# tky823/audio_source_separation

Measured on AMD Instinct MI355X. Metric: ILRMA iterations/sec (4ch, F=1025, T=4096), higher is better.
Workload: dtype f64; 1 GPU; gauss_ilrma_ip update_once, M=4 F=1025 T=4096 K=4, normalize=power, loss off; utterances_per_gpu=1, power_statistic=covariance, parallelism=utterance-sharded x1, no data-path collective

## Files before the change

audio_source_separation_amd/_lib.py:

```python
import ctypes
import os

import torch

_HERE = os.path.dirname(os.path.abspath(__file__))
LIB_PATH = os.environ.get("ASSX_LIB_PATH") or os.path.join(_HERE, "csrc", "libassx.so")

F32, F64 = 0, 1
W_NONE, W_NT, W_NFT = 0, 1, 2
IVA_LAPLACE, IVA_GAUSS = 0, 1
NMF_EUC, NMF_KL, NMF_IS_MM, NMF_IS_ME = 0, 1, 2, 3
NMF_T, NMF_CAUCHY_NAIVE, NMF_CAUCHY_MM, NMF_CAUCHY_ME, NMF_CAUCHY_MM_FAST = 4, 5, 6, 7, 8
STATUS_SINGULAR, STATUS_COND_REJECT = 1, 2
SPATIAL_IP, SPATIAL_ISS, SPATIAL_IP2 = 0, 1, 2

_vp = ctypes.c_void_p
_i = ctypes.c_int
_d = ctypes.c_double
_sz = ctypes.c_size_t
_ll = ctypes.c_longlong

SIGNATURES = {
    "assx_ctx_create": (_i, [_i, ctypes.POINTER(_vp)]),
    "assx_ctx_destroy": (_i, [_vp]),
    "assx_last_error": (ctypes.c_char_p, [_vp]),
    "assx_version": (ctypes.c_char_p, []),
    "assx_workspace_bytes": (_sz, [_i, _i, _i, _i, _i, _i]),
    "assx_launch_order": (_i, [_i, _i, _i, _i, _vp, _i]),
    "assx_nmf_partition_query": (_i, [_i, _i, _i, _i, _i, _i, _i, _vp]),
    "assx_demix": (_i, [_vp, _vp, _vp, _vp, _vp, _i, _i, _i, _i, _i, _vp]),
    "assx_cov_accumulate": (_i, [_vp, _vp, _vp, _i, _d, _vp, _vp, _i, _i, _i, _i, _i, _i, _vp]),
    "assx_ip_update": (_i, [_vp, _vp, _vp, _d, _vp, _i, _i, _i, _i, _vp]),
    "assx_ilrma_source_update": (_i, [_vp, _vp, _vp, _vp, _vp, _d, _d, ctypes.c_uint, _vp, _vp, _i, _i, _i, _i, _i, _i, _vp]),
    "assx_ilrma_expand_partitioned": (_i, [_vp, _vp, _vp, _vp, _vp, _vp, _i, _i, _i, _i, _i, _i, _vp]),
    "assx_ilrma_source_update_partitioned": (_i, [_vp, _vp, _vp, _vp, _vp, _vp, _vp, _vp, _d, _vp, _i, _i, _i, _i, _i, _i, _vp]),
    "assx_ilrma_normalize_power_bins_partitioned": (_i, [_vp, _vp, _vp, _vp, _vp, _d, _vp, _i, _i, _i, _i, _i, _vp]),
    "assx_ilrma_spatial_update": (_i, [_vp, _i, _i, _i, _vp, _vp, _vp, _vp, _d, _d, _d, _vp, _vp, _vp, _vp, _vp, _i, _i, _i, _i, _i, _i, _vp]),
    "assx_ip2_update": (_i, [_vp, _vp, _vp, _d, _vp, _i, _i, _i, _i, _i, _i, _vp]),
    "assx_iss_update": (_i, [_vp, _vp, _vp, _i, _i, _i, _i, _i, _vp]),
    "assx_ilrma_cov_partials": (_i, [_vp, _vp, _vp, _vp, _d, _d, _vp, _i, _i, _i, _i, _i, _i, _vp]),
    "assx_demix_power": (_i, [_vp, _vp, _vp, _vp, _vp, _i, _i, _i, _i, _i, _vp]),
    "assx_power_from_cov": (_i, [_vp, _vp, _vp, _vp, _vp, _i, _i, _i, _i, _vp]),
    "assx_ilrma_normalize_power": (_i, [_vp, _vp, _vp, _vp, _d, _d, _i, _i, _i, _i, _i, _vp]),
    "assx_ilrma_normalize_power_bins": (_i, [_vp, _vp, _vp, _vp, _d, _d, _i, _i, _i, _i, _i, _vp]),
    "assx_ilrma_normalize_pb": (_i, [_vp, _vp, _vp, _vp, _d, _i, _i, _i, _i, _i, _vp]),
    "assx_ilrma_loss": (_i, [_vp, _vp, _vp, _vp, _vp, _d, _d, _vp, _vp, _i, _i, _i, _i, _i, _i, _vp]),
    "assx_tilrma_source_update": (_i, [_vp, _vp, _vp, _vp, _vp, _d, _d, _vp, _i, _i, _i, _i, _i, _i, _vp]),
    "assx_tilrma_spatial_update": (_i, [_vp, _vp, _vp, _vp, _vp, _d, _d, _vp, _vp, _vp, _vp, _vp, _i, _i, _i, _i, _i, _i, _vp]),
    "assx_tilrma_loss": (_i, [_vp, _vp, _vp, _vp, _vp, _d, _d, _vp, _vp, _i, _i, _i, _i, _i, _i, _vp]),
    "assx_auxiva_weights": (_i, [_vp, _vp, _vp, _i, _d, _vp, _vp, _vp, _i, _i, _i, _i, _i, _vp]),
    "assx_auxiva_spatial_update": (_i, [_vp, _i, _i, _i, _vp, _vp, _vp, _d, _d, _vp, _vp, _vp, _i, _i, _i, _i, _i, _vp]),
    "assx_idlma_space_update": (_i, [_vp, _vp, _vp, _vp, _d, _d, _d, _vp, _vp, _vp, _i, _i, _i, _i, _i, _vp]),
    "assx_fastmnmf_update_diagonalizer": (_i, [_vp, _vp, _vp, _vp, _vp, _d, _d, _vp, _vp, _vp, _i, _i, _i, _i, _i, _i, _vp]),
    "assx_fastmnmf_workspace_bytes": (_sz, [_i, _i, _i, _i, _i, _i, _i]),
    "assx_fastmnmf_project": (_i, [_vp, _vp, _vp, _vp, _vp, _vp, _d, _vp, _vp, _i, _i, _i, _i, _i, _i, _i, _vp]),
    "assx_fastmnmf_update_nmf": (_i, [_vp, _vp, _vp, _vp, _d, _vp, _i, _i, _i, _i, _i, _i, _i, _vp]),
    "assx_fastmnmf_update_scm": (_i, [_vp, _vp, _vp, _vp, _d, _vp, _i, _i, _i, _i, _i, _i, _i, _vp]),
    "assx_fastmnmf_update_diagonalizer_model": (_i, [_vp, _vp, _vp, _vp, _vp, _vp, _d, _d, _vp, _vp, _i, _i, _i, _i, _i, _i,
                                                     _i, _vp]),
    "assx_fastmnmf_normalize_power": (_i, [_vp, _vp, _vp, _vp, _vp, _d, _i, _i, _i, _i, _i, _i, _i, _vp]),
    "assx_fastmnmf_separate": (_i, [_vp, _vp, _vp, _vp, _vp, _vp, _i, _d, _vp, _vp, _i, _i, _i, _i, _i, _i, _i, _vp]),
# ... 76 lines not shown
```

audio_source_separation_amd/csrc/assx_bss.hip:

```cpp
#include "assx_common.hpp"
#include "assx_small_linalg.hpp"
#include "assx_stream.hpp"
#include "assx_group_linalg.hpp"
#include "assx_partition.hpp"
#include "assx_cov_wide.hpp"
#include "assx_cov_mfma.hpp"
#include "assx_nmf_internal.hpp"
#include "assx_widem.hpp"

using namespace assx;

namespace {

constexpr int REDUCE_THREADS = 256;

template <typename R, int M>
__device__ __forceinline__ void load_filter(const Cx<R>* __restrict__ W, size_t bf, Cx<R> (&w)[M][M]) {
  const Cx<R>* p = W + bf * (M * M);
#pragma unroll
  for (int n = 0; n < M; ++n)
#pragma unroll
    for (int m = 0; m < M; ++m) w[n][m] = p[n * M + m];
}

// ... 837 lines not shown
#endif
    }
  } else if (dtype == ASSX_F32) {
#if !defined(ASSX_DEV_ONLY_M4_F64)
    switch (M) {
#if !defined(ASSX_DEV_ONLY_M4_F32)
      case 2: return fn(float(), IntC<2>());
      case 3: return fn(float(), IntC<3>());
#endif
      case 4: return fn(float(), IntC<4>());
    }
#endif
  } else {
    return fail(ctx, ASSX_E_ARG, "dtype must be ASSX_F32 or ASSX_F64, got %d", dtype);
  }
  return fail(ctx, ASSX_E_UNSUPPORTED,
              "this entry point supports 2 <= M <= 4 channels, got M=%d (5 <= M <= 32 runs on the wide-channel path of the "
              "model entry points; more than 32 channels are not supported)", M);
}

#define CHECK_COMMON(ctx, B, M, F, T)                                                        \
  ASSX_REQUIRE_CTX(ctx);                              \
  ASSX_REQUIRE(ctx, (B) >= 1 && (M) >= 1 && (F) >= 1 && (T) >= 1, ASSX_E_ARG,                 \
               "invalid sizes B=%d M=%d F=%d T=%d", (B), (M), (F), (T));                       \
  ASSX_REQUIRE(ctx, (long long)(M) * (F) * (T) < (1LL << 28) && (long long)(B) * (F) * (((T) + 31) / 32 + 1) < (1LL << 31), \
               ASSX_E_UNSUPPORTED,                                                                                       \
               "utterance too large: buffer offsets are 32-bit, one utterance must stay below 4 GiB in complex128 "     \
               "(M*F*T < 2^28) and B*F*T/32 below 2^31")

inline unsigned blocks_for(size_t n, int bs) { return (unsigned)((n + bs - 1) / bs); }

inline unsigned set_launch_order(FlatPart& fp, int B, int rev) {
  static const int on = lab_int("ASSX_UTT_ORDER", 1);
  if (!on || B < 2) {
    fp.Gp = 0;
    fp.rev = 0;
    return (unsigned)fp.G;
  }
  fp.Gp = (fp.Gu + N_XCD - 1) / N_XCD * N_XCD;
  fp.rev = rev ? 1 : 0;
  return (unsigned)B * (unsigned)fp.Gp;
}
inline unsigned stream_grid(assx_ctx* ctx, FlatPart& fp, int B) {
  return set_launch_order(fp, B, B >= 2 ? (int)(ctx->stream_pass++ & 1u) : 0);
}

template <typename R, int M>
int run_cov_partial(assx_ctx* ctx, int wk, const void* X, const void* r, const void* Tb, const void* V, int K,
                    double domain, double eps, void* ws, int B, int F, int T, hipStream_t st, FlatPart* fp_out) {
  CovArgs<R> a;
  a.d = Dims{B, F, T, K};
  a.fp = flat_cov(B, F, T, wk == WK_NONE ? 1 : cov_lane_split<R, M>());
  a.eps = (R)eps;
  a.p2d = make_pow(2.0 / domain);
  *fp_out = a.fp;
  dim3 grid(stream_grid(ctx, a.fp, B));
  const bool d2 = a.p2d.mode == POW_ID;
#define COV_LAUNCH(WKV, K4V, D2V, LSV, DXV, DWV, MW) \
  hipLaunchKernelGGL((cov_stream_kernel<R, M, WKV, K4V, D2V, LSV, DXV, DWV, MW>), grid, dim3(64), 0, st, \
                     (const Cx<R>*)X, (const R*)r, (const R*)Tb, (const R*)V, (R*)ws, a)
  constexpr int LSX = cov_lane_split<R, M>();
  switch (wk) {
    case WK_NONE: COV_LAUNCH(WK_NONE, true, true, 1, 4, 1, 1); break;
    case WK_NT: COV_LAUNCH(WK_NT, true, true, LSX, 3, 1, 2); break;
    case WK_NFT: COV_LAUNCH(WK_NFT, true, true, LSX, 3, 1, 2); break;
    default:
      if (K <= KU) {
        constexpr size_t vlds = (size_t)VDMA_SLOTS * VTileDma<R, M * KU>::TILE_BYTES;
#if ASSX_LAB
        static const int vdma = lab_int("ASSX_COV_VDMA", 1);
        if (!vdma) {
          if (d2) COV_LAUNCH(WK_TV, true, true, LSX, (sizeof(R) == 8 ? 2 : 4), 1, 2);
          else COV_LAUNCH(WK_TV, true, false, LSX, 2, 1, 1);
        } else
#endif
        if (d2)
          hipLaunchKernelGGL((cov_stream_kernel<R, M, WK_TV, true, true, 1, 2, 1, 2, true>), grid, dim3(64), vlds, st,
                             (const Cx<R>*)X, (const R*)r, (const R*)Tb, (const R*)V, (R*)ws, a);
        else
          hipLaunchKernelGGL((cov_stream_kernel<R, M, WK_TV, true, false, 1, 2, 1, 1, true>), grid, dim3(64), vlds, st,
                             (const Cx<R>*)X, (const R*)r, (const R*)Tb, (const R*)V, (R*)ws, a);
      }
      else if (d2) COV_LAUNCH(WK_TV, false, true, LSX, 4, 1, 1);
      else COV_LAUNCH(WK_TV, false, false, LSX, 2, 1, 1);
  }
#undef COV_LAUNCH
  ASSX_LAUNCH_CHECK(ctx, "cov_stream_kernel");
  return 0;
}

template <typename R, int M>
int run_cov(assx_ctx* ctx, int wk, const void* X, const void* r, const void* Tb, const void* V, int K, double domain,
            double eps, void* U, void* ws, int B, int F, int T, hipStream_t st) {
  FlatPart fp;
  int rc = run_cov_partial<R, M>(ctx, wk, X, r, Tb, V, K, domain, eps, ws, B, F, T, st, &fp);
  if (rc) return rc;
  const int N = (wk == WK_NONE) ? 1 : M;
  const size_t total = (size_t)B * N * F * M * M;
  hipLaunchKernelGGL((cov_stream_finalize_kernel<R, M>), dim3(blocks_for(total, 256)), dim3(256), 0, st, (const R*)ws,
                     (Cx<R>*)U, B, N, F, fp, (R)(1.0 / (double)T));
  ASSX_LAUNCH_CHECK(ctx, "cov_stream_finalize_kernel");
  return 0;
}

template <typename R, int M>
int run_ip(assx_ctx* ctx, const void* U, const void* part, FlatPart fp, int T, void* W, const void* C, double* pw,
           double thr, int32_t* status, int B, int F, hipStream_t st, double den_floor = 0.0, int wb = 1) {
  constexpr int GPW = WAVE / next_pow2_c(M * M);
#if ASSX_LAB
  const int par = lab_int("ASSX_IP_PAR", 0);
  if (par) {
    const dim3 gp(blocks_for((size_t)B * F, GPW / M)), bp(64);
    if (part)
      hipLaunchKernelGGL((ip_par_kernel<R, M, true>), gp, bp, 0, st, (const Cx<R>*)nullptr, (const R*)part, fp,
// ... 29 lines not shown
                       (double)T, (Cx<R>*)W, (const Cx<R>*)C, pw, B, F);
  ASSX_LAUNCH_CHECK(ctx, "iss_group_kernel");
  return 0;
}

template <typename R, int M>
int run_ip2(assx_ctx* ctx, const void* U, const void* part, FlatPart fp, int T, void* W, const void* C, double* pw,
            double thr, int32_t* status, int B, int F, int pm, int pn, hipStream_t st) {
  constexpr int GPW = WAVE / next_pow2_c(M * M);
  const dim3 grid(blocks_for((size_t)B * F, GPW)), block(64);
  if (part)
    hipLaunchKernelGGL((ip2_group_kernel<R, M, true>), grid, block, 0, st, (const Cx<R>*)nullptr, (const R*)part, fp,
                       1.0 / (double)T, (Cx<R>*)W, (const Cx<R>*)C, pw, thr, status, B, F, pm, pn);
  else
    hipLaunchKernelGGL((ip2_group_kernel<R, M, false>), grid, block, 0, st, (const Cx<R>*)U, (const R*)nullptr, fp, 1.0,
                       (Cx<R>*)W, (const Cx<R>*)C, pw, thr, status, B, F, pm, pn);
  ASSX_LAUNCH_CHECK(ctx, "ip2_group_kernel");
  return 0;
}

template <typename R, int MM>
int run_basis_partial(assx_ctx* ctx, const void* X, const void* W, const void* Tb, const void* V, double domain,
                      double eps, void* ws, int B, int F, int T, int K, hipStream_t st, FlatPart* fp_out,
                      double nu = -1.0 ,
                      double* lpart = nullptr , int lstride = 0) {
  NmfArgs<R> a;
  a.nu = (R)nu;
  a.d = Dims{B, F, T, K};
  a.eps = (R)eps;
  a.p1 = make_pow((domain + 2.0) / domain);
  a.fp = flat_basis(B, F, T);
  *fp_out = a.fp;
  const bool d2 = a.p1.mode == POW_SQUARE, k4 = K <= KU;
  const dim3 gb(stream_grid(ctx, a.fp, B)), bb(64);
#define BASIS_LAUNCH(K4V, D2V, DXV, DWV, MW) \
  hipLaunchKernelGGL((basis_stream_kernel<R, MM, K4V, D2V, DXV, DWV, MW>), gb, bb, 0, st, (const Cx<R>*)X, \
                     (const Cx<R>*)W, (const R*)Tb, (const R*)V, (R*)ws, a)
  constexpr size_t vlds = (size_t)VDMA_SLOTS * VTileDma<R, MM * KU>::TILE_BYTES;
#define BASIS_VD(D2V, MW, TDV) \
  hipLaunchKernelGGL((basis_stream_vd_kernel<R, MM, D2V, 2, MW, TDV>), gb, bb, vlds, st, (const Cx<R>*)X, \
                     (const Cx<R>*)W, (const R*)Tb, (const R*)V, (R*)ws, a, (double*)nullptr, 0)
#if ASSX_LAB
  static const int vdma = lab_int("ASSX_BASIS_VDMA", 1);
  if (k4 && !vdma) {
    if (nu >= 0.0) hipLaunchKernelGGL((basis_stream_kernel<R, MM, true, true, 3, 1, 1, true>), gb, bb, 0, st, (const Cx<R>*)X,
                                      (const Cx<R>*)W, (const R*)Tb, (const R*)V, (R*)ws, a);
    else if (d2) BASIS_LAUNCH(true, true, 3, 1, 2);
    else BASIS_LAUNCH(true, false, 2, 1, 1);
  } else
#endif
  if (nu >= 0.0) {
    if (k4) BASIS_VD(true, 2, true);
    else hipLaunchKernelGGL((basis_stream_kernel<R, MM, false, true, 3, 1, 1, true>), gb, bb, 0, st, (const Cx<R>*)X,
                            (const Cx<R>*)W, (const R*)Tb, (const R*)V, (R*)ws, a);
  } else if (k4) {
    if (d2 && lpart)
      hipLaunchKernelGGL((basis_stream_vd_kernel<R, MM, true, 2, 2, false, true>), gb, bb, vlds, st, (const Cx<R>*)X,
                         (const Cx<R>*)W, (const R*)Tb, (const R*)V, (R*)ws, a, lpart, lstride);
    else if (d2) BASIS_VD(true, 2, false);
    else BASIS_VD(false, 1, false);
  } else if (d2) BASIS_LAUNCH(false, true, 3, 1, 1);
  else BASIS_LAUNCH(false, false, 2, 1, 1);
#undef BASIS_VD
#undef BASIS_LAUNCH
  ASSX_LAUNCH_CHECK(ctx, "basis_stream_kernel");
  return 0;
}

template <typename R, int MM>
int run_act_partial(assx_ctx* ctx, const void* X, const void* W, const void* Tb, const void* V, double domain,
                    double eps, void* ws, int B, int F, int T, int K, hipStream_t st, FlatPart* fp_out,
                    double nu = -1.0) {
  NmfArgs<R> a;
  a.nu = (R)nu;
  a.d = Dims{B, F, T, K};
  a.eps = (R)eps;
  a.p1 = make_pow((domain + 2.0) / domain);
  a.fp = flat_act(B, F, T);
  *fp_out = a.fp;
  const bool d2 = a.p1.mode == POW_SQUARE, k4 = K <= KU;
  const dim3 ga(stream_grid(ctx, a.fp, B)), ba(64 * ACT_NH);
#define ACT_LAUNCH(K4V, D2V, DXV, MW) \
  hipLaunchKernelGGL((act_stream_kernel<R, MM, K4V, D2V, DXV, MW>), ga, ba, 0, st, (const Cx<R>*)X, (const Cx<R>*)W, \
                     (const R*)Tb, (const R*)V, (R*)ws, a)
#define ACT_VD(D2V, DXV, MW, TDV) \
  hipLaunchKernelGGL((act_stream_vd_kernel<R, MM, D2V, DXV, MW, TDV>), ga, ba, 0, st, (const Cx<R>*)X, (const Cx<R>*)W, \
                     (const R*)Tb, (const R*)V, (R*)ws, a)
#if ASSX_LAB
  static const int vdma = lab_int("ASSX_ACT_VDMA", 1);
  if (k4 && !vdma) {
    if (nu >= 0.0) hipLaunchKernelGGL((act_stream_kernel<R, MM, true, true, 3, 1, true>), ga, ba, 0, st, (const Cx<R>*)X,
                                      (const Cx<R>*)W, (const R*)Tb, (const R*)V, (R*)ws, a);
    else if (d2) ACT_LAUNCH(true, true, (sizeof(R) == 8 ? 3 : 4), 2);
    else ACT_LAUNCH(true, false, 2, 1);
  } else
#endif
// ... 92 lines not shown
      *fp_out = fw;
      return 0;
    }
    hipLaunchKernelGGL((cov_wide_finalize_kernel<R, MM>), dim3(blocks_for((size_t)B * MM * F * MM * MM, 256)), dim3(256),
                       0, st, (const R*)ws, (Cx<R>*)U_dense, B, F, fw, (R)(1.0 / (double)T));
    ASSX_LAUNCH_CHECK(ctx, "cov_wide_finalize_kernel");
    *fp_out = fw;
    *dense = true;
    return 0;
  }
  R* rv = (R*)((char*)ws + L.map);
  const dim3 grid(blocks_for(T, 256), blocks_for(F, WIDE_FB), B * MM);
  if (p2d.mode == POW_ID)
    hipLaunchKernelGGL((source_variance_map_kernel<R, true>), grid, dim3(256), 0, st, (const R*)Tb, (const R*)V, rv, F, T,
                       K, p2d);
  else
    hipLaunchKernelGGL((source_variance_map_kernel<R, false>), grid, dim3(256), 0, st, (const R*)Tb, (const R*)V, rv, F,
                       T, K, p2d);
  ASSX_LAUNCH_CHECK(ctx, "source_variance_map_kernel");
  return run_cov_partial<R, MM>(ctx, WK_NFT, X, rv, nullptr, nullptr, 1, 2.0, eps, ws, B, F, T, st, fp_out);
}

}

extern "C" {

int assx_launch_order(int B, int F, int T, int reverse, int* ranges, int capacity) {
  if (B < 1 || F < 1 || T < 1) return ASSX_E_ARG;
  FlatPart fp = flat_cov(B, F, T, 1);
  const int grid = (int)set_launch_order(fp, B, reverse);
  if (ranges) {
    if (capacity < grid) return ASSX_E_ARG;
    for (int bid = 0; bid < grid; ++bid) ranges[bid] = workgroup_range(bid, grid, fp);
  }
  return grid;
}

size_t assx_workspace_bytes(int B, int M, int F, int T, int K, int dtype) {
  if (B < 1 || M < 1 || F < 1 || T < 1) return 0;
  if (widem::handles(M)) return widem::workspace_bytes(B, M, F, T, K, dtype);
  return ws_layout(B, M, F, T, K, dtype).total;
}

int assx_demix(assx_ctx* ctx, const void* X, const void* W, const void* scale, void* Y, int B, int M, int F, int T,
               int dtype, void* stream) {
  CHECK_COMMON(ctx, B, M, F, T);
  ASSX_REQUIRE(ctx, X && W && Y, ASSX_E_NULL, "assx_demix: NULL array");
  if (widem::handles(M)) return widem::demix(ctx, X, W, scale, Y, B, M, F, T, dtype, (hipStream_t)stream);
  hipStream_t st = (hipStream_t)stream;
  return dispatch_rm(ctx, dtype, M, [&](auto rt, auto mt) -> int {
    using R = decltype(rt);
    constexpr int MM = decltype(mt)::value;
    dim3 grid(blocks_for(T, 256), F, B);
    hipLaunchKernelGGL((demix_kernel<R, MM>), grid, dim3(256), 0, st, (const Cx<R>*)X, (const Cx<R>*)W,
                       (const Cx<R>*)scale, (Cx<R>*)Y, Dims{B, F, T, 0});
    ASSX_LAUNCH_CHECK(ctx, "demix_kernel");
    return 0;
  });
}

int assx_ilrma_power_map(assx_ctx* ctx, const void* X, const void* W, void* P, int B, int M, int F, int T, int dtype,
                         void* stream) {
  CHECK_COMMON(ctx, B, M, F, T);
  ASSX_REQUIRE(ctx, X && W && P, ASSX_E_NULL, "assx_ilrma_power_map: NULL array");
  hipStream_t st = (hipStream_t)stream;
  if (widem::handles(M)) return widem::power_map(ctx, X, W, P, B, M, F, T, dtype, st);
// ... 877 lines not shown
```

audio_source_separation_amd/csrc/assx_stream.hpp:

```cpp
#pragma once
#include <cstdlib>
#include "assx_common.hpp"

namespace assx {

enum { WK_NONE = 0, WK_NT = 1, WK_NFT = 2, WK_TV = 3 };

constexpr int KU = 4;

struct Dims {
  int B, F, T, K;
};

struct FlatPart {
  long long NB;
  int len;
  int L;
  int G;
  int S;
  int Gu;
  int Ju;
  int P;
  int Gp;
  int rev;
};

inline FlatPart make_flat(int B, long long NB, int len, long long G_target) {
  FlatPart p;
  p.Gp = 0;
  p.rev = 0;
  p.NB = NB;
  p.len = len;
  p.Ju = (int)(NB / len);
  p.P = 0;
  long long G = G_target < NB ? G_target : NB;
  if (G < 1) G = 1;
  const long long parts = G / p.Ju;
  static const bool align = lab_int("ASSX_ALIGN", 1) != 0;
  if (align && parts >= 1 && parts <= len && p.Ju * parts * 100 >= G * 97) {
    p.L = (int)((len + parts - 1) / parts);
    p.P = (len + p.L - 1) / p.L;
    p.Gu = p.Ju * p.P;
    p.G = B * p.Gu;
    p.S = 1;
    return p;
  }
  p.L = (int)((NB + G - 1) / G);
  p.Gu = (int)((NB + p.L - 1) / p.L);
  p.G = B * p.Gu;
  p.S = (p.L + len - 2) / len + 1;
  return p;
}

__host__ __device__ __forceinline__ bool flat_local(const FlatPart& fp, unsigned gl, unsigned& lo, unsigned& n) {
  const unsigned L = (unsigned)fp.L;
  if (fp.P > 0) {
    const unsigned grp = gl / (unsigned)fp.P, part = gl - grp * (unsigned)fp.P, len = (unsigned)fp.len;
    const unsigned off = part * L;
    if (off >= len) return false;
    lo = grp * len + off;
    n = off + L < len ? L : len - off;
    return true;
  }
// ... 28 lines not shown
    g_hi = g_lo + (fp.len + fp.L - 1) / fp.L - 1;
    return;
  }
  const unsigned lo = jl * (unsigned)fp.len;
  g_lo = b * fp.Gu + (int)(lo / (unsigned)fp.L);
  g_hi = b * fp.Gu + (int)((lo + (unsigned)fp.len - 1u) / (unsigned)fp.L);
}
__host__ __device__ __forceinline__ int flat_slot(const FlatPart& fp, long long j, int g) {
  if (fp.P > 0) return 0;
  const int b = g / fp.Gu, gl = g - b * fp.Gu;
  return (int)(j - (long long)b * fp.Ju) - (int)(((unsigned)gl * (unsigned)fp.L) / (unsigned)fp.len);
}

struct Cursor {
  int b, f, tb;
};
__device__ __forceinline__ void advance(Cursor& c, int TBk, int F) {
  if (++c.tb == TBk) {
    c.tb = 0;
    if (++c.f == F) {
      c.f = 0;
      ++c.b;
    }
  }
}

constexpr int N_XCD = 8;
__host__ __device__ __forceinline__ int xcd_local_range(int bid, int G) {
  const int x = bid % N_XCD, j = bid / N_XCD;
  const int q = G / N_XCD, r = G % N_XCD;
  return x * q + (x < r ? x : r) + j;
}

__host__ __device__ __forceinline__ int workgroup_range(int bid, int grid, const FlatPart& fp) {
  if (fp.Gp == 0) return xcd_local_range(bid, grid);
  const int Gp = fp.Gp, B = grid / Gp;
  int b = bid / Gp;
  const int r = bid - b * Gp;
  const int x = r % N_XCD, j = r / N_XCD;
  const int q = fp.Gu / N_XCD, rem = fp.Gu % N_XCD;
  const int cnt = q + (x < rem ? 1 : 0);
  if (j >= cnt) return -1;
  const int first = x * q + (x < rem ? x : rem);
  if (fp.rev) {
    b = B - 1 - b;
    return b * fp.Gu + first + (cnt - 1 - j);
  }
  return b * fp.Gu + first + j;
}


template <typename R, int NROW>
struct VTileDma {
  static constexpr int LPR = WAVE * (int)sizeof(R) / 16;
  static constexpr int RPI = WAVE / LPR;
  static constexpr int NI = NROW / RPI;
  static constexpr int ROW_BYTES = WAVE * (int)sizeof(R);
  static constexpr int TILE_BYTES = NROW * ROW_BYTES;
  static constexpr int NP = NROW / 2;
  static_assert(NROW % RPI == 0 && NROW % 2 == 0 && (NP == 4 || NP == 6 || NP == 8), "tile geometry");
  unsigned vro[NI];

  __device__ __forceinline__ void init(int lane, int K, unsigned t_row) {
    const int grp = lane / LPR, piece = lane % LPR;
#pragma unroll
    for (int j = 0; j < NI; ++j) {
      const int rho = j * RPI + grp;
      const int n = rho / KU, kk = rho % KU;
      vro[j] = (unsigned)(n * K + (kk < K ? kk : K - 1)) * t_row + (unsigned)piece * 16u;
    }
  }
  __device__ __forceinline__ void issue(BufRsrc rv, unsigned char* slot, unsigned soff) const {
#if defined(__HIP_DEVICE_COMPILE__)
#pragma unroll
    for (int j = 0; j < NI; ++j)
      __builtin_amdgcn_raw_ptr_buffer_load_lds(rv, (__attribute__((address_space(3))) void*)(slot + j * RPI * ROW_BYTES),
                                               16, (int)vro[j], (int)soff, 0, 0);
#endif
  }
};

// ... 58 lines not shown
      "ds_read2st64_b32 %0, %4 offset0:0 offset1:1\n\tds_read2st64_b32 %1, %4 offset0:2 offset1:3\n\t"
      "ds_read2st64_b32 %2, %4 offset0:4 offset1:5\n\tds_read2st64_b32 %3, %4 offset0:6 offset1:7\n\t"
      "s_waitcnt lgkmcnt(0)"
      : "=&v"(o[0]), "=&v"(o[1]), "=&v"(o[2]), "=&v"(o[3])
      : "v"(addr)
      : "memory");
}

constexpr int VDMA_SLOTS = 2;

template <int M>
__host__ __device__ constexpr int herm_pair_base(int m, int l) {
  return M + 2 * (m * M - m * (m + 1) / 2 + (l - m - 1));
}

template <typename R>
struct CovArgs {
  Dims d;
  FlatPart fp;
  R eps;
  PowSpec p2d;
};

#ifndef STREAM_TRACE
#define STREAM_TRACE 0
#endif
#if STREAM_TRACE && !defined(ASSX_PROBE_BUILD)
#error "STREAM_TRACE adds a debug entry point and stamps: build it with -DASSX_PROBE_BUILD into a probe library, never into libassx.so"
#endif
#if STREAM_TRACE
__device__ unsigned long long g_stream_trace[8 * 4096];
#endif

template <typename R, int M, int WK, bool K4, bool D2, int LS, int DXT, int DWT, int MINW = 1, bool VDMA = false>
__global__ void __launch_bounds__(64, MINW)
    cov_stream_kernel(const Cx<R>* __restrict__ X, const R* __restrict__ rw ,
                      const R* __restrict__ Tb , const R* __restrict__ V ,
                      R* __restrict__ part, CovArgs<R> a) {
  constexpr int N = (WK == WK_NONE) ? 1 : M;
  static_assert(N % LS == 0 && DXT % DWT == 0, "lane split / ring depths");
  constexpr int FB = WAVE / LS;
  constexpr int SPL = N / LS;
  constexpr int HM = M * M;
  constexpr int NACC = SPL * HM;
  constexpr int NV = next_pow2_c(NACC);
  static_assert(NV <= FB, "accumulators per lane must not exceed the lanes of a group");
  constexpr int NWV = (WK == WK_TV) ? KU : 1;
  constexpr bool VD = VDMA && WK == WK_TV && K4;
  static_assert(!VD || (LS == 1 && DXT >= 2), "the LDS ring path walks whole 64-frame blocks");
  using VT = VTileDma<R, (VD ? SPL * KU : 16)>;
  extern __shared__ __attribute__((aligned(16))) unsigned char vlds[];
  const int lane = threadIdx.x & (WAVE - 1);
  const int fl = lane & (FB - 1);
  const int s0 = (lane / FB) * SPL;
  const int F = a.d.F, T = a.d.T, K = a.d.K, TBk = a.fp.len;
  const size_t FT = (size_t)F * T;
  const int g = workgroup_range((int)blockIdx.x, (int)gridDim.x, a.fp);
  if (g < 0) return;
  Cursor cc;
  int nblk;
  if (!flat_start(a.fp, g, cc.b, cc.f, cc.tb, nblk)) return;
#if STREAM_TRACE
  if (lane == 0 && g < 4096) {
    g_stream_trace[8 * g + 0] = __builtin_amdgcn_s_memrealtime();
    g_stream_trace[8 * g + 2] = (unsigned long long)(__builtin_amdgcn_s_getreg((31 << 11) | 20) & 0xf) | ((unsigned long long)nblk << 8) |
                                ((unsigned long long)blockIdx.x << 32);
    g_stream_trace[8 * g + 4] = __builtin_amdgcn_s_getreg((31 << 11) | 4);
    g_stream_trace[8 * g + 5] = __builtin_readcyclecounter();
  }
#endif
  const int bf_first = cc.b * F + cc.f;
  Cursor px = cc, pw = cc;
  const bool ragged = (T % FB) != 0;

  R acc[NV];
#pragma unroll
  for (int i = 0; i < NV; ++i) acc[i] = 0;

  const unsigned x_row = (unsigned)FT * (unsigned)sizeof(Cx<R>);
  const unsigned t_row = (unsigned)T * (unsigned)sizeof(R);

  auto issue_x = [&](const Cursor& c, Vec2<R>(&x)[M], R after) {
    const int t = c.tb * FB + fl;
    const unsigned tc = (unsigned)(t < T ? t : T - 1);
    const BufRsrc rx = make_rsrc(X + (size_t)c.b * M * FT);
    const unsigned voff = order_after(((unsigned)c.f * (unsigned)T + tc) * (unsigned)sizeof(Cx<R>), after);
    unsigned so = 0;
    const unsigned step = sgpr_opaque(x_row);
#pragma unroll
    for (int m = 0; m < M; ++m) {
// ... 423 lines not shown
            }
            tv = floor_eps<R>(tv, a.eps);
            if (TD) P = t_harmonic<R>(P, tv, a.nu);
            R inv = fast_rcp(tv);
            R D = D2 ? P * inv * inv : P / powspec<R>(tv, a.p1);
            if (ragged && t >= T) {
              inv = 0;
              D = 0;
            }
#pragma unroll
            for (int kk = 0; kk < KU; ++kk) {
              acc[(n * KU + kk) * 2 + 0] = fma(D, v[n][kk], acc[(n * KU + kk) * 2 + 0]);
              acc[(n * KU + kk) * 2 + 1] = fma(inv, v[n][kk], acc[(n * KU + kk) * 2 + 1]);
            }
          }

          if (cc.tb == 0 || !more) {
            const R tot = wave_reduce_scatter<R, NV>(acc);
            const int i = scatter_index<NV>();
            const int slot = cur.b * F + cur.f - bf_first;
            const int n = i / (2 * KU), k = k0 + (i >> 1) % KU;
            if (scatter_leader<NV>() && i < NACC && k < K)
              part[(((size_t)g * a.fp.S + slot) * N + n) * (size_t)(2 * K) + k * 2 + (i & 1)] = tot;
#pragma unroll
            for (int q = 0; q < NV; ++q) acc[q] = 0;
            if (more) load_rows(cc);
          }
        }
      }
    }
  }
}

template <typename R, int M, bool D2, int DXT, int MINW, bool TD, bool LOSS = false>
__global__ void __launch_bounds__(64, MINW)
    basis_stream_vd_kernel(const Cx<R>* __restrict__ X, const Cx<R>* __restrict__ W, const R* __restrict__ Tb,
                           const R* __restrict__ V, R* __restrict__ part, NmfArgs<R> a, double* __restrict__ lpart,
                           int lstride) {
  static_assert(!LOSS || (D2 && !TD), "the fused loss is the domain-2 Gaussian one");
  constexpr int N = M;
  constexpr int NACC = N * KU * 2;
  constexpr int NV = next_pow2_c(NACC);
  static_assert(NV <= WAVE && DXT >= 2, "accumulators / ring depth");
  using VT = VTileDma<R, N * KU>;
  extern __shared__ __attribute__((aligned(16))) unsigned char vlds[];
  const int lane = threadIdx.x & (WAVE - 1);
  const int F = a.d.F, T = a.d.T, K = a.d.K, TBk = a.fp.len;
  const size_t FT = (size_t)F * T;
  const int g = workgroup_range((int)blockIdx.x, (int)gridDim.x, a.fp);
  if (g < 0) return;
  Cursor cc;
  int nblk;
  if (!flat_start(a.fp, g, cc.b, cc.f, cc.tb, nblk)) return;
  const int bf_first = cc.b * F + cc.f;
  Cursor px = cc, pw = cc;
  const unsigned x_row = (unsigned)FT * (unsigned)sizeof(Cx<R>);
  const unsigned t_row = (unsigned)T * (unsigned)sizeof(R);

  R acc[NV];
#pragma unroll
  for (int i = 0; i < NV; ++i) acc[i] = 0;
  double lacc = 0.0, lm = 1.0;
  int le = 0;

  auto issue_x_tied = [&](const Cursor& c, Vec2<R>(&x)[M]) {
    const int t = c.tb * WAVE + lane;
    const unsigned tc = (unsigned)(t < T ? t : T - 1);
    const buf_u4 rx = make_rsrc_words(X + (size_t)c.b * M * FT, ~(size_t)0);
    const unsigned voff = ((unsigned)c.f * (unsigned)T + tc) * (unsigned)sizeof(Cx<R>);
    unsigned so = 0;
    const unsigned step = sgpr_opaque(x_row);
#pragma unroll
    for (int m = 0; m < M; ++m) {
      buf_ldv_tied(x[m], rx, voff, so);
      so += step;
    }
  };
  VT vt;
  vt.init(lane, K, t_row);
  const unsigned vlds0 =
      (unsigned)(size_t)(__attribute__((address_space(3))) void*)vlds + (unsigned)lane * (unsigned)sizeof(R);
  auto issue_vtile = [&](const Cursor& c, int slot) {
// ... 372 lines not shown
            }
            const R r = floor_eps<R>(D2 ? tv : powspec<R>(tv, p2d), a.eps);
            if (TD) tprod *= fma((double)((R)2 * fast_rcp(a.nu)), (double)(cabs2(y) * fast_rcp(r)), 1.0);
            else term += (double)(cabs2(y) * fast_rcp(r));
            rprod *= (double)r;
          }
          if (t < T) {
            acc += term;
            int e;
            lm = frexp(lm * rprod, &e);
            le += e;
            if (TD) {
              tm = frexp(tm * tprod, &e);
              te += e;
            }
          }
          if (cc.tb == 0 && it + 1 < nblk) load_rows(cc);
        }
      }
    }
  }
  acc += (double)le * 0.6931471805599453 + log(lm);
  if (TD) acc += (1.0 + 0.5 * (double)a.nu) * ((double)te * 0.6931471805599453 + log(tm));
  acc = wave_allreduce_sum<double>(acc);
  if (lane == 0) lpart[(size_t)b * lstride + g] = acc;
}

template <typename R, int M, bool D2, int DXT, int MINW, bool TD>
__global__ void __launch_bounds__(64, MINW)
    loss_stream_vd_kernel(const Cx<R>* __restrict__ X, const Cx<R>* __restrict__ W, const R* __restrict__ Tb,
                          const R* __restrict__ V, double* __restrict__ lpart, int lstride, NmfArgs<R> a, PowSpec p2d) {
  constexpr int N = M;
  static_assert(DXT >= 2, "ring depth");
  using VT = VTileDma<R, N * KU>;
  extern __shared__ __attribute__((aligned(16))) unsigned char vlds[];
  const int lane = threadIdx.x & (WAVE - 1);
  const int F = a.d.F, T = a.d.T, K = a.d.K, TBk = a.fp.len;
  const size_t FT = (size_t)F * T;
  const int g = xcd_local_range((int)blockIdx.x, (int)gridDim.x), b = blockIdx.y;
  long long q0, q1;
  flat_range(a.fp, g, q0, q1);
  double acc = 0.0;
  double lm = 1.0, tm = 1.0;
  int le = 0, te = 0;
  if (q0 < q1) {
    const int nblk = (int)(q1 - q0);
    Cursor cc;
    cc.f = (int)(q0 / TBk);
    cc.tb = (int)(q0 - (long long)cc.f * TBk);
    cc.b = b;
    Cursor px = cc, pw = cc;
    const unsigned x_row = (unsigned)FT * (unsigned)sizeof(Cx<R>);
    const unsigned t_row = (unsigned)T * (unsigned)sizeof(R);
    const buf_u4 rx = make_rsrc_words(X + (size_t)b * M * FT, ~(size_t)0);
    const BufRsrc rv = make_rsrc_sized(V + (size_t)b * N * K * T, (size_t)(a.d.B - b) * N * K * T * sizeof(R));
    auto issue_x_tied = [&](const Cursor& c, Vec2<R>(&x)[M]) {
      const int t = c.tb * WAVE + lane;
      const unsigned tc = (unsigned)(t < T ? t : T - 1);
      const unsigned voff = ((unsigned)c.f * (unsigned)T + tc) * (unsigned)sizeof(Cx<R>);
      unsigned so = 0;
      const unsigned step = sgpr_opaque(x_row);
#pragma unroll
      for (int m = 0; m < M; ++m) {
        buf_ldv_tied(x[m], rx, voff, so);
        so += step;
      }
// ... 485 lines not shown
```

include/assx.h:

```cpp
#ifndef ASSX_H
#define ASSX_H

#include <stddef.h>
#include <stdint.h>

#ifdef __cplusplus
extern "C" {
#endif

#define ASSX_VERSION_STRING "assx 0.1.0 (gfx950)"

enum { ASSX_F32 = 0, ASSX_F64 = 1 };

enum { ASSX_E_ARG = -1, ASSX_E_UNSUPPORTED = -2, ASSX_E_NULL = -3 };

enum {
  ASSX_STATUS_SINGULAR = 1,
  ASSX_STATUS_COND_REJECT = 2
};

enum { ASSX_W_NONE = 0, ASSX_W_NT = 1, ASSX_W_NFT = 2 };

enum { ASSX_IVA_LAPLACE = 0, ASSX_IVA_GAUSS = 1 };

enum { ASSX_SPATIAL_IP = 0, ASSX_SPATIAL_ISS = 1, ASSX_SPATIAL_IP2 = 2 };

enum { ASSX_NMF_EUC = 0, ASSX_NMF_KL = 1, ASSX_NMF_IS_MM = 2, ASSX_NMF_IS_ME = 3,
       ASSX_NMF_T = 4,
       ASSX_NMF_CAUCHY_NAIVE = 5,
       ASSX_NMF_CAUCHY_MM = 6,
       ASSX_NMF_CAUCHY_ME = 7,
       ASSX_NMF_CAUCHY_MM_FAST = 8,
       ASSX_NMF_T_RAW = 9            };

typedef struct assx_ctx assx_ctx;

int assx_ctx_create(int device, assx_ctx** ctx);
int assx_ctx_destroy(assx_ctx* ctx);
const char* assx_last_error(const assx_ctx* ctx);
const char* assx_version(void);
size_t assx_workspace_bytes(int B, int M, int F, int T, int K, int dtype);
int assx_launch_order(int B, int F, int T, int reverse, int* ranges, int capacity);

int assx_demix(assx_ctx* ctx, const void* X, const void* W, const void* scale, void* Y,
               int B, int M, int F, int T, int dtype, void* stream);

int assx_cov_accumulate(assx_ctx* ctx, const void* X, const void* r, int r_kind, double eps, void* U,
                        void* ws, int B, int M, int N, int F, int T, int dtype, void* stream);

int assx_ip_update(assx_ctx* ctx, const void* U, void* W, double threshold, int32_t* status,
                   int B, int M, int F, int dtype, void* stream);

int assx_iss_update(assx_ctx* ctx, const void* U, void* W, int n_frames, int B, int M, int F, int dtype, void* stream);
int assx_ip2_update(assx_ctx* ctx, const void* U, void* W, double threshold, int32_t* status, int pair_m, int pair_n,
                    int B, int M, int F, int dtype, void* stream);

int assx_ilrma_source_update(assx_ctx* ctx, const void* X, const void* W, void* Tb, void* V,
                             double domain, double eps, unsigned source_mask, double* loss_prev, void* ws,
                             int B, int M, int F, int T, int K, int dtype, void* stream);

int assx_ilrma_expand_partitioned(assx_ctx* ctx, const void* Z, const void* Tb, const void* V, void* Teff, void* Veff,
                                  int B, int M, int F, int T, int K, int dtype, void* stream);
int assx_ilrma_source_update_partitioned(assx_ctx* ctx, const void* X, const void* W, void* Z, void* Tb, void* V,
                                         void* Teff, void* Veff, double eps, void* ws,
                                         int B, int M, int F, int T, int K, int dtype, void* stream);
int assx_ilrma_normalize_power_bins_partitioned(assx_ctx* ctx, void* W, void* Z, void* Tb, const double* power_bins,
                                                double eps, void* ws, int B, int M, int F, int K, int dtype,
                                                void* stream);

int assx_ilrma_spatial_update(assx_ctx* ctx, int spatial, int pair_m, int pair_n, const void* X, void* W, const void* Tb, const void* V,
                              double domain, double eps, double threshold, void* U_out,
                              const void* C, double* power_bins,
                              int32_t* status, void* ws,
                              int B, int M, int F, int T, int K, int dtype, void* stream);

// ... 149 lines not shown
```

Baseline: 5568 iterations/s.

## Group four phase-aligned waves per workgroup in cov and basis stream kernels

Lets the covariance and basis streaming kernels launch four waves per workgroup. Each wave takes a range chosen so that the waves in one group share the same activation-tile phase, and each wave gets its own LDS tile ring. A new launch-slot mapping (wave_range) and a phase-group setup compute those ranges, and a wave-order query is exported for inspection. The aim is better CU packing and tile sharing among co-resident waves. The cost is more LDS per workgroup and a more involved range mapping.

New measurement: 5655 iterations/s (median of 6 runs). 1.02x the previous value.

```diff
diff --git a/audio_source_separation_amd/_lib.py b/audio_source_separation_amd/_lib.py
--- a/audio_source_separation_amd/_lib.py
+++ b/audio_source_separation_amd/_lib.py
@@ -27,6 +27,7 @@
     "assx_version": (ctypes.c_char_p, []),
     "assx_workspace_bytes": (_sz, [_i, _i, _i, _i, _i, _i]),
     "assx_launch_order": (_i, [_i, _i, _i, _i, _vp, _i]),
+    "assx_wave_order": (_i, [_i, _i, _i, _i, _vp, _vp, _i]),
     "assx_nmf_partition_query": (_i, [_i, _i, _i, _i, _i, _i, _i, _vp]),
     "assx_demix": (_i, [_vp, _vp, _vp, _vp, _vp, _i, _i, _i, _i, _i, _vp]),
     "assx_cov_accumulate": (_i, [_vp, _vp, _vp, _i, _d, _vp, _vp, _i, _i, _i, _i, _i, _i, _vp]),
diff --git a/audio_source_separation_amd/csrc/assx_bss.hip b/audio_source_separation_amd/csrc/assx_bss.hip
--- a/audio_source_separation_amd/csrc/assx_bss.hip
+++ b/audio_source_separation_amd/csrc/assx_bss.hip
@@ -893,17 +893,22 @@
 
 inline unsigned set_launch_order(FlatPart& fp, int B, int rev) {
   static const int on = lab_int("ASSX_UTT_ORDER", 1);
+  const int U = fp.Q > 0 ? fp.Wu : fp.Gu;
   if (!on || B < 2) {
     fp.Gp = 0;
     fp.rev = 0;
-    return (unsigned)fp.G;
-  }
-  fp.Gp = (fp.Gu + N_XCD - 1) / N_XCD * N_XCD;
+    return (unsigned)B * (unsigned)U;
+  }
+  fp.Gp = (U + N_XCD - 1) / N_XCD * N_XCD;
   fp.rev = rev ? 1 : 0;
   return (unsigned)B * (unsigned)fp.Gp;
 }
 inline unsigned stream_grid(assx_ctx* ctx, FlatPart& fp, int B) {
   return set_launch_order(fp, B, B >= 2 ? (int)(ctx->stream_pass++ & 1u) : 0);
+}
+inline int stream_phase_groups(FlatPart& fp) {
+  static const int nw = lab_int("ASSX_PHASE_NW", PHASE_NW);
+  return set_phase_groups(fp, nw >= 2 ? PHASE_NW : 1, (long long)CHIP_CUS * 8);
 }
 
 template <typename R, int M>
@@ -915,6 +920,12 @@
   a.eps = (R)eps;
   a.p2d = make_pow(2.0 / domain);
   *fp_out = a.fp;
+  bool vd = wk == WK_TV && K <= KU;
+#if ASSX_LAB
+  static const int vdma = lab_int("ASSX_COV_VDMA", 1);
+  vd = vd && vdma;
+#endif
+  const int nw = vd ? stream_phase_groups(a.fp) : 1;
   dim3 grid(stream_grid(ctx, a.fp, B));
   const bool d2 = a.p2d.mode == POW_ID;
 #define COV_LAUNCH(WKV, K4V, D2V, LSV, DXV, DWV, MW) \
@@ -928,19 +939,21 @@
     default:
       if (K <= KU) {
         constexpr size_t vlds = (size_t)VDMA_SLOTS * VTileDma<R, M * KU>::TILE_BYTES;
+#define COV_VD(D2V, MW, NWV) \
+  hipLaunchKernelGGL((cov_stream_kernel<R, M, WK_TV, true, D2V, 1, 2, 1, MW, true, NWV>), grid, dim3(64 * NWV), \
+                     vlds * NWV, st, (const Cx<R>*)X, (const R*)r, (const R*)Tb, (const R*)V, (R*)ws, a)
 #if ASSX_LAB
-        static const int vdma = lab_int("ASSX_COV_VDMA", 1);
-        if (!vdma) {
+        if (!vd) {
           if (d2) COV_LAUNCH(WK_TV, true, true, LSX, (sizeof(R) == 8 ? 2 : 4), 1, 2);
           else COV_LAUNCH(WK_TV, true, false, LSX, 2, 1, 1);
         } else
 #endif
-        if (d2)
-          hipLaunchKernelGGL((cov_stream_kernel<R, M, WK_TV, true, true, 1, 2, 1, 2, true>), grid, dim3(64), vlds, st,
-                             (const Cx<R>*)X, (const R*)r, (const R*)Tb, (const R*)V, (R*)ws, a);
-        else
-          hipLaunchKernelGGL((cov_stream_kernel<R, M, WK_TV, true, false, 1, 2, 1, 1, true>), grid, dim3(64), vlds, st,
-                             (const Cx<R>*)X, (const R*)r, (const R*)Tb, (const R*)V, (R*)ws, a);
+        if (nw > 1) {
+          if (d2) COV_VD(true, 2, PHASE_NW);
+          else COV_VD(false, 1, PHASE_NW);
+        } else if (d2) COV_VD(true, 2, 1);
+        else COV_VD(false, 1, 1);
+#undef COV_VD
       }
       else if (d2) COV_LAUNCH(WK_TV, false, true, LSX, 4, 1, 1);
       else COV_LAUNCH(WK_TV, false, false, LSX, 2, 1, 1);
@@ -1036,17 +1049,28 @@
   a.fp = flat_basis(B, F, T);
   *fp_out = a.fp;
   const bool d2 = a.p1.mode == POW_SQUARE, k4 = K <= KU;
+  bool vd = k4;
+#if ASSX_LAB
+  static const int vdma = lab_int("ASSX_BASIS_VDMA", 1);
+  vd = vd && vdma;
+#endif
+  const int nw = vd ? stream_phase_groups(a.fp) : 1;
   const dim3 gb(stream_grid(ctx, a.fp, B)), bb(64);
 #define BASIS_LAUNCH(K4V, D2V, DXV, DWV, MW) \
   hipLaunchKernelGGL((basis_stream_kernel<R, MM, K4V, D2V, DXV, DWV, MW>), gb, bb, 0, st, (const Cx<R>*)X, \
                      (const Cx<R>*)W, (const R*)Tb, (const R*)V, (R*)ws, a)
   constexpr size_t vlds = (size_t)VDMA_SLOTS * VTileDma<R, MM * KU>::TILE_BYTES;
-#define BASIS_VD(D2V, MW, TDV) \
-  hipLaunchKernelGGL((basis_stream_vd_kernel<R, MM, D2V, 2, MW, TDV>), gb, bb, vlds, st, (const Cx<R>*)X, \
-                     (const Cx<R>*)W, (const R*)Tb, (const R*)V, (R*)ws, a, (double*)nullptr, 0)
+#define BASIS_VD_NW(D2V, MW, TDV, LOSSV, NWV, LP, LS) \
+  hipLaunchKernelGGL((basis_stream_vd_kernel<R, MM, D2V, 2, MW, TDV, LOSSV, NWV>), gb, dim3(64 * NWV), \
+                     vlds * NWV, st, (const Cx<R>*)X, (const Cx<R>*)W, (const R*)Tb, (const R*)V, (R*)ws, \
+                     a, LP, LS)
+#define BASIS_VD(D2V, MW, TDV)                                                      \
+  do {                                                                              \
+    if (nw > 1) BASIS_VD_NW(D2V, MW, TDV, false, PHASE_NW, (double*)nullptr, 0);    \
+    else BASIS_VD_NW(D2V, MW, TDV, false, 1, (double*)nullptr, 0);                  \
+  } while (0)
 #if ASSX_LAB
-  static const int vdma = lab_int("ASSX_BASIS_VDMA", 1);
-  if (k4 && !vdma) {
+  if (k4 && !vd) {
     if (nu >= 0.0) hipLaunchKernelGGL((basis_stream_kernel<R, MM, true, true, 3, 1, 1, true>), gb, bb, 0, st, (const Cx<R>*)X,
                                       (const Cx<R>*)W, (const R*)Tb, (const R*)V, (R*)ws, a);
     else if (d2) BASIS_LAUNCH(true, true, 3, 1, 2);
@@ -1058,14 +1082,15 @@
     else hipLaunchKernelGGL((basis_stream_kernel<R, MM, false, true, 3, 1, 1, true>), gb, bb, 0, st, (const Cx<R>*)X,
                             (const Cx<R>*)W, (const R*)Tb, (const R*)V, (R*)ws, a);
   } else if (k4) {
-    if (d2 && lpart)
-      hipLaunchKernelGGL((basis_stream_vd_kernel<R, MM, true, 2, 2, false, true>), gb, bb, vlds, st, (const Cx<R>*)X,
-                         (const Cx<R>*)W, (const R*)Tb, (const R*)V, (R*)ws, a, lpart, lstride);
-    else if (d2) BASIS_VD(true, 2, false);
+    if (d2 && lpart) {
+      if (nw > 1) BASIS_VD_NW(true, 2, false, true, PHASE_NW, lpart, lstride);
+      else BASIS_VD_NW(true, 2, false, true, 1, lpart, lstride);
+    } else if (d2) BASIS_VD(true, 2, false);
     else BASIS_VD(false, 1, false);
   } else if (d2) BASIS_LAUNCH(false, true, 3, 1, 1);
   else BASIS_LAUNCH(false, false, 2, 1, 1);
 #undef BASIS_VD
+#undef BASIS_VD_NW
 #undef BASIS_LAUNCH
   ASSX_LAUNCH_CHECK(ctx, "basis_stream_kernel");
   return 0;
@@ -1224,6 +1249,21 @@
   if (ranges) {
     if (capacity < grid) return ASSX_E_ARG;
     for (int bid = 0; bid < grid; ++bid) ranges[bid] = workgroup_range(bid, grid, fp);
+  }
+  return grid;
+}
+
+int assx_wave_order(int B, int F, int T, int reverse, int* waves, int* ranges, int capacity) {
+  if (B < 1 || F < 1 || T < 1 || !waves) return ASSX_E_ARG;
+  FlatPart fp = flat_cov(B, F, T, 1);
+  const int nw = stream_phase_groups(fp);
+  const int grid = (int)set_launch_order(fp, B, reverse);
+  *waves = nw;
+  if (ranges) {
+    if (capacity < grid * nw) return ASSX_E_ARG;
+    for (int bid = 0; bid < grid; ++bid)
+      for (int w = 0; w < nw; ++w)
+        ranges[bid * nw + w] = nw > 1 ? wave_range<PHASE_NW>(bid, grid, w, fp) : workgroup_range(bid, grid, fp);
   }
   return grid;
 }
diff --git a/audio_source_separation_amd/csrc/assx_stream.hpp b/audio_source_separation_amd/csrc/assx_stream.hpp
--- a/audio_source_separation_amd/csrc/assx_stream.hpp
+++ b/audio_source_separation_amd/csrc/assx_stream.hpp
@@ -23,12 +23,16 @@
   int P;
   int Gp;
   int rev;
+  int Q;
+  int Wu;
 };
 
 inline FlatPart make_flat(int B, long long NB, int len, long long G_target) {
   FlatPart p;
   p.Gp = 0;
   p.rev = 0;
+  p.Q = 0;
+  p.Wu = 0;
   p.NB = NB;
   p.len = len;
   p.Ju = (int)(NB / len);
@@ -123,21 +127,66 @@
   return x * q + (x < r ? x : r) + j;
 }
 
-__host__ __device__ __forceinline__ int workgroup_range(int bid, int grid, const FlatPart& fp) {
-  if (fp.Gp == 0) return xcd_local_range(bid, grid);
-  const int Gp = fp.Gp, B = grid / Gp;
+__host__ __device__ __forceinline__ int launch_slot(int bid, int grid, int U, int Gp, int rev) {
+  if (Gp == 0) return xcd_local_range(bid, grid);
+  const int B = grid / Gp;
   int b = bid / Gp;
   const int r = bid - b * Gp;
   const int x = r % N_XCD, j = r / N_XCD;
-  const int q = fp.Gu / N_XCD, rem = fp.Gu % N_XCD;
+  const int q = U / N_XCD, rem = U % N_XCD;
   const int cnt = q + (x < rem ? 1 : 0);
   if (j >= cnt) return -1;
   const int first = x * q + (x < rem ? x : rem);
-  if (fp.rev) {
+  if (rev) {
     b = B - 1 - b;
-    return b * fp.Gu + first + (cnt - 1 - j);
-  }
-  return b * fp.Gu + first + j;
+    return b * U + first + (cnt - 1 - j);
+  }
+  return b * U + first + j;
+}
+__host__ __device__ __forceinline__ int workgroup_range(int bid, int grid, const FlatPart& fp) {
+  return launch_slot(bid, grid, fp.Gu, fp.Gp, fp.rev);
+}
+
+constexpr int PHASE_NW = 4;
+__host__ __device__ __forceinline__ int phase_chunks(int Gu, int Q, int NW) { return ((Gu + Q - 1) / Q + NW - 1) / NW; }
+inline int phase_period(const FlatPart& fp) {
+  if (fp.P > 0) return fp.P;
+  int a = fp.L, b = fp.len;
+  while (b) {
+    const int t = a % b;
+    a = b;
+    b = t;
+  }
+  return fp.len / a;
+}
+inline int set_phase_groups(FlatPart& fp, int NW, long long slots) {
+  fp.Q = 0;
+  fp.Wu = 0;
+  if (NW < 2) return 1;
+  const int Q = phase_period(fp);
+  if (Q >= fp.Gu) return 1;
+  const long long Wu = (long long)Q * phase_chunks(fp.Gu, Q, NW);
+  if (Wu * NW > slots) return 1;
+  fp.Q = Q;
+  fp.Wu = (int)Wu;
+  return NW;
+}
+template <int NW>
+__host__ __device__ __forceinline__ int wave_range(int bid, int grid, int wave, const FlatPart& fp) {
+  if (NW == 1) return workgroup_range(bid, grid, fp);
+  const int u = launch_slot(bid, grid, fp.Wu, fp.Gp, fp.rev);
+  if (u < 0) return -1;
+  const int b = u / fp.Wu, ul = u - b * fp.Wu;
+  const int chunk = ul / fp.Q, cls = ul - chunk * fp.Q;
+  const int gl = cls + (chunk * NW + wave) * fp.Q;
+  return gl < fp.Gu ? b * fp.Gu + gl : -1;
+}
+__device__ __forceinline__ int wave_in_workgroup() {
+#if defined(__HIP_DEVICE_COMPILE__)
+  return __builtin_amdgcn_readfirstlane((int)(threadIdx.x / WAVE));
+#else
+  return 0;
+#endif
 }
 
 
@@ -262,8 +311,8 @@
 __device__ unsigned long long g_stream_trace[8 * 4096];
 #endif
 
-template <typename R, int M, int WK, bool K4, bool D2, int LS, int DXT, int DWT, int MINW = 1, bool VDMA = false>
-__global__ void __launch_bounds__(64, MINW)
+template <typename R, int M, int WK, bool K4, bool D2, int LS, int DXT, int DWT, int MINW = 1, bool VDMA = false, int NW = 1>
+__global__ void __launch_bounds__(64 * NW, MINW)
     cov_stream_kernel(const Cx<R>* __restrict__ X, const R* __restrict__ rw ,
                       const R* __restrict__ Tb , const R* __restrict__ V ,
                       R* __restrict__ part, CovArgs<R> a) {
@@ -278,14 +327,18 @@
   constexpr int NWV = (WK == WK_TV) ? KU : 1;
   constexpr bool VD = VDMA && WK == WK_TV && K4;
   static_assert(!VD || (LS == 1 && DXT >= 2), "the LDS ring path walks whole 64-frame blocks");
+  static_assert(NW == 1 || VD, "wave groups exist to share the activation tiles of the LDS ring path");
+  static_assert(!VD || DXT >= VDMA_SLOTS, "the counted waits assume an X ring at least as deep as the tile ring");
   using VT = VTileDma<R, (VD ? SPL * KU : 16)>;
-  extern __shared__ __attribute__((aligned(16))) unsigned char vlds[];
+  extern __shared__ __attribute__((aligned(16))) unsigned char vlds_wg[];
+  const int wv = NW > 1 ? wave_in_workgroup() : 0;
+  unsigned char* const vlds = vlds_wg + wv * (VDMA_SLOTS * VT::TILE_BYTES);
   const int lane = threadIdx.x & (WAVE - 1);
   const int fl = lane & (FB - 1);
   const int s0 = (lane / FB) * SPL;
   const int F = a.d.F, T = a.d.T, K = a.d.K, TBk = a.fp.len;
   const size_t FT = (size_t)F * T;
-  const int g = workgroup_range((int)blockIdx.x, (int)gridDim.x, a.fp);
+  const int g = wave_range<NW>((int)blockIdx.x, (int)gridDim.x, wv, a.fp);
   if (g < 0) return;
   Cursor cc;
   int nblk;
@@ -775,8 +828,8 @@
   }
 }
 
-template <typename R, int M, bool D2, int DXT, int MINW, bool TD, bool LOSS = false>
-__global__ void __launch_bounds__(64, MINW)
+template <typename R, int M, bool D2, int DXT, int MINW, bool TD, bool LOSS = false, int NW = 1>
+__global__ void __launch_bounds__(64 * NW, MINW)
     basis_stream_vd_kernel(const Cx<R>* __restrict__ X, const Cx<R>* __restrict__ W, const R* __restrict__ Tb,
                            const R* __restrict__ V, R* __restrict__ part, NmfArgs<R> a, double* __restrict__ lpart,
                            int lstride) {
@@ -785,12 +838,15 @@
   constexpr int NACC = N * KU * 2;
   constexpr int NV = next_pow2_c(NACC);
   static_assert(NV <= WAVE && DXT >= 2, "accumulators / ring depth");
+  static_assert(DXT >= VDMA_SLOTS, "the counted waits assume an X ring at least as deep as the tile ring");
   using VT = VTileDma<R, N * KU>;
-  extern __shared__ __attribute__((aligned(16))) unsigned char vlds[];
+  extern __shared__ __attribute__((aligned(16))) unsigned char vlds_wg[];
+  const int wv = NW > 1 ? wave_in_workgroup() : 0;
+  unsigned char* const vlds = vlds_wg + wv * (VDMA_SLOTS * VT::TILE_BYTES);
   const int lane = threadIdx.x & (WAVE - 1);
   const int F = a.d.F, T = a.d.T, K = a.d.K, TBk = a.fp.len;
   const size_t FT = (size_t)F * T;
-  const int g = workgroup_range((int)blockIdx.x, (int)gridDim.x, a.fp);
+  const int g = wave_range<NW>((int)blockIdx.x, (int)gridDim.x, wv, a.fp);
   if (g < 0) return;
   Cursor cc;
   int nblk;
@@ -1229,6 +1285,7 @@
                           const R* __restrict__ V, double* __restrict__ lpart, int lstride, NmfArgs<R> a, PowSpec p2d) {
   constexpr int N = M;
   static_assert(DXT >= 2, "ring depth");
+  static_assert(DXT >= VDMA_SLOTS, "the counted waits assume an X ring at least as deep as the tile ring");
   using VT = VTileDma<R, N * KU>;
   extern __shared__ __attribute__((aligned(16))) unsigned char vlds[];
   const int lane = threadIdx.x & (WAVE - 1);
diff --git a/include/assx.h b/include/assx.h
--- a/include/assx.h
+++ b/include/assx.h
@@ -41,6 +41,7 @@
 const char* assx_version(void);
 size_t assx_workspace_bytes(int B, int M, int F, int T, int K, int dtype);
 int assx_launch_order(int B, int F, int T, int reverse, int* ranges, int capacity);
+int assx_wave_order(int B, int F, int T, int reverse, int* waves, int* ranges, int capacity);
 
 int assx_demix(assx_ctx* ctx, const void* X, const void* W, const void* scale, void* Y,
                int B, int M, int F, int T, int dtype, void* stream);
```
